# dmsuehir/unet_distributed

Measured on AMD Instinct MI355X. Metric: images/sec (whole node) 2D UNet BraTS 128×128×4 at 1/2/4/8 MI355X; Dice parity, higher is better.
Workload: dtype bf16; 1 GPU; model=unet2d-transposed (base 32, depth 4, 7760385 params), global_batch=1024, per_gpu_batch=1024, img_size=128, in_channels=4, parallelism=dp1, backend=native

## Files before the change

### unet_distributed_amd/csrc/kernels/conv_epilogue.h

```cpp
#pragma once
#include "common.h"
#include "conv_params.h"

namespace unet {

struct PixCoord {
  int n, d, h, w;
};

__device__ __forceinline__ PixCoord decompose(int q, int OD, int OH, int OW) {
  PixCoord c;
  c.w = q % OW;
  int t = q / OW;
  c.h = t % OH;
  t /= OH;
  c.d = t % OD;
  c.n = t / OD;
  return c;
}

enum { EPI_GENERIC = 0, EPI_FWD = 1, EPI_DGRAD = 2, EPI_STATS = 3, EPI_DGRAD_NORM = 4 };

template <int BM, int BN, int NTHR = 256>
constexpr int epi_lds_bytes() {
// ... 1 lines not shown
}

__device__ __forceinline__ size_t route_pix(const ConvFwdParams& p, int q, uint32_t& rk) {
  const int g = q / p.OW, w = q - g * p.OW;
  if (p.OD > 1) {
    const int s = g / p.OH, h = g - s * p.OH;
    rk = ((uint32_t)(s & 1) << 2) | ((uint32_t)(h & 1) << 1) | (uint32_t)(w & 1);
    return ((size_t)(s >> 1) * (p.OH >> 1) + (h >> 1)) * (p.OW >> 1) + (w >> 1);
  }
  rk = ((uint32_t)(g & 1) << 1) | (uint32_t)(w & 1);
  return (size_t)(g >> 1) * (p.OW >> 1) + (w >> 1);
}
__device__ __forceinline__ bool route_hit(uint32_t cw, int e, uint32_t rk, bool d3) {
  const uint32_t k = d3 ? (cw >> (3 * e)) & 7u : (cw >> (2 * e)) & 3u;
  return k == rk && ((cw >> (24 + e)) & 1u);
}

__host__ __device__ inline const char* conv_norm_epi_check(const ConvFwdParams& p) {
  if (!p.stats && !p.nz) return nullptr;
  if (!p.stats) return "conv_fwd: nz (dgrad-norm epilogue) needs a stats buffer";
  if (p.relu || p.shuffle || p.drop_rate > 0.f || p.out_scale != 1.f || p.D1 != p.Cout || p.mask1 || p.mask2 ||
      p.head_w || p.relu_bits || p.mask_bits || (p.route_gy && !p.nz))
    return "conv_fwd: statistics epilogue takes no ReLU / dropout / shuffle / scale / split / mask / head";
  if (p.nz && (p.bias || !p.na || !p.nc || p.npix <= 0 || p.mask_scale1 != 1.f || (p.ncs != 0 && p.ncs != p.Cout)))
    return "conv_fwd: dgrad-norm epilogue needs na / nc / npix, no bias";
  return nullptr;
}

__host__ __device__ inline int conv_epi_mode(const ConvFwdParams& p) {
  if (p.nz) return EPI_DGRAD_NORM;
  if (p.stats) return EPI_STATS;
  if (p.shuffle || p.drop_rate > 0.f || p.out_scale != 1.f) return EPI_GENERIC;
  if (p.relu && p.D1 == p.Cout && !p.mask1 && !p.mask2 && p.mask_scale1 == 1.f) return EPI_FWD;
  if (!p.relu && !p.bias) return EPI_DGRAD;
  return EPI_GENERIC;
}

template <int WM>
struct LinearTiles {
  __device__ static int base(int wm, int i) { return wm * WM + i * 16; }
};
template <int W, int RW, int TC, int NCS>
struct StripTiles {
  __device__ static int base(int wave, int i) {
    return ((wave / NCS) * RW + i / TC) * W + (wave % NCS) * 16 * TC + (i % TC) * 16;
  }
};

constexpr int kWaitVm0 = 0x0f70, kWaitLgkm0 = 0xc07f;
__device__ __forceinline__ void lds_barrier() {
  asm volatile("" ::: "memory");
  __builtin_amdgcn_s_waitcnt(kWaitLgkm0);
  __builtin_amdgcn_s_barrier();
  asm volatile("" ::: "memory");
}

template <int TN>
struct EpiConst {
  float bias[TN][4];
  float hw[8];
  float hb;
};

struct HeadWsum {
  float s[3][8];
  float u, v, w;
};
struct HeadT {
  float t[8];
  bool on;
};

template <int BM, int BN, int NTHR>
__device__ __forceinline__ void epi_mask_bits_load(const ConvFwdParams& p, const int m0, const int n0, const int tid,
                                                   uint32_t (&mb)[BM * (BN / 8) / NTHR]) {
  constexpr int CPR = BN / 8, NIT = BM * CPR / NTHR, RPI = NTHR / CPR;
  static_assert(BM * CPR % NTHR == 0 && NTHR % CPR == 0, "whole chunk passes");
  const int co = n0 + (tid % CPR) * 8, ml0 = tid / CPR;
#pragma unroll
  for (int it = 0; it < NIT; ++it)
    mb[it] = ((const uint8_t*)p.mask1)[((size_t)(m0 + ml0 + it * RPI) * p.D1 + co) >> 3];
}

template <int BM, int BN, int WM, int WN, int TM, int TN, int NTHR, int EPI = EPI_GENERIC,
          class MapM = LinearTiles<WM>, int SEGW = 0, int TROW = 0>
__device__ __forceinline__ HeadWsum conv_epilogue(const ConvFwdParams p, f32x4 (&acc)[TM][TN], char* smem,
                                                  const int m0, const int n0, const int M, const int wm,
                                                  const int wn, const int lane, const int tid,
                                                  const int pitch = 0, const int col0 = 0, const int stat_row = 0,
                                                  const EpiConst<TN>* ec = nullptr, const HeadT ht = HeadT{},
                                                  const uint32_t* pmb = nullptr) {
  HeadWsum hws;
#pragma unroll
  for (int k = 0; k < 3; ++k)
#pragma unroll
    for (int e = 0; e < 8; ++e) hws.s[k][e] = 0.f;
  hws.u = hws.v = hws.w = 0.f;
  auto qof = [&](int ml) -> int {
    if constexpr (SEGW > 0) return (m0 + ml / SEGW) * pitch + col0 + (ml % SEGW);
    else return m0 + ml;
  };
  constexpr bool ESWZ = BN == 32;
  constexpr int EPI_STRIDE = ESWZ ? 64 : (BN + 4) * 2;
  auto eoff = [](const int ml, const int chunk) -> int {
    return ESWZ ? ml * 64 + 16 * (chunk ^ ((ml >> 2) & 3)) : ml * EPI_STRIDE + 16 * chunk;
  };
  auto ehalf = [](const int ml, const int nl) -> int {
    return ESWZ ? ml * 64 + 16 * ((nl >> 3) ^ ((ml >> 2) & 3)) + ((2 * (nl & 7)) ^ (8 * ((ml >> 1) & 1)))
                : ml * EPI_STRIDE + 2 * nl;
  };
  auto eread = [&](const int ml, const int chunk) -> u32x4 {
    if constexpr (ESWZ) {
      const u32x4 v = *(const u32x4*)(smem + eoff(ml, chunk));
      return ((ml >> 1) & 1) ? (u32x4){v[2], v[3], v[0], v[1]} : v;
    } else {
      const u32x2 lo = *(const u32x2*)(smem + eoff(ml, chunk));
      const u32x2 hi = *(const u32x2*)(smem + eoff(ml, chunk) + 8);
      return (u32x4){lo[0], lo[1], hi[0], hi[1]};
    }
  };
  char* E = smem;
  float* SP = (float*)(smem + BM * EPI_STRIDE);
  constexpr bool G = EPI == EPI_GENERIC;
  constexpr bool kNormG = EPI == EPI_DGRAD_NORM;
  const bool kRelu = G ? (p.relu != 0) : (EPI == EPI_FWD);
  const bool kBias = EPI != EPI_DGRAD && !kNormG && p.bias;
  const bool kDrop = G && p.drop_rate > 0.f;
  constexpr bool kStats = EPI == EPI_STATS;
  const bool kShuffle = G && p.shuffle;
  constexpr bool kMaskScale = EPI == EPI_GENERIC || EPI == EPI_DGRAD;
  const float inv_keep = p.drop_rate > 0.f ? 1.f / (1.f - p.drop_rate) : 1.f;
  const uint32_t drop_thr = (uint32_t)(p.drop_rate * 4294967296.0);
  const uint32_t seed = (kDrop && p.seed_ptr) ? *p.seed_ptr : p.seed;
  const int Dtb = kShuffle ? (p.Cout >> p.shuffle) : p.Cout;
#pragma unroll
  for (int j = 0; j < TN; ++j) {
    const int nl = wn * WN + j * 16 + (lane >> 4) * 4;
    const int n = n0 + nl;
    float bsv[4], msc[4];
#pragma unroll
    for (int r = 0; r < 4; ++r) {
      bsv[r] = ec ? ec->bias[j][r] : (kBias ? p.bias[kShuffle ? (n + r) % Dtb : n + r] : 0.f);
      msc[r] = kMaskScale ? ((n + r < p.D1) ? p.mask_scale1 : p.mask_scale2) : 1.f;
    }
    if constexpr (EPI == EPI_FWD) {
      const f32x2 b01 = {bsv[0], bsv[1]}, b23 = {bsv[2], bsv[3]};
#pragma unroll
      for (int i = 0; i < TM; ++i) {
        const int ml = MapM::base(wm, i) + (lane & 15);
        f32x2 a01 = (f32x2){acc[i][j][0], acc[i][j][1]} + b01;
        f32x2 a23 = (f32x2){acc[i][j][2], acc[i][j][3]} + b23;
        u32x2 pk;
        pk[0] = relu2h(pack2h(a01[0], a01[1]));
        pk[1] = relu2h(pack2h(a23[0], a23[1]));
        *(u32x2*)(E + ehalf(ml, nl)) = pk;
      }
      continue;
    }
#pragma unroll
    for (int i = 0; i < TM; ++i) {
      const int ml = MapM::base(wm, i) + (lane & 15);
      const int q = qof(ml);
      float v[4];
#pragma unroll
      for (int r = 0; r < 4; ++r) {
        float x = G ? acc[i][j][r] * p.out_scale + bsv[r] : acc[i][j][r] + bsv[r];
        if (kRelu) x = fmaxf(x, 0.f);
        if (kDrop) {
          const uint32_t h = drop_hash((uint64_t)q * p.Cout + n + r + p.drop_idx0, seed, p.salt);
          x = (h >= drop_thr) ? x * inv_keep : 0.f;
        }
        if (kMaskScale) x *= msc[r];
        v[r] = x;
      }
      u32x2 pk;
      pk[0] = pack2h(v[0], v[1]);
      pk[1] = pack2h(v[2], v[3]);
      *(u32x2*)(E + ehalf(ml, nl)) = pk;
    }
  }
  if (pmb)
    lds_barrier();
  else
    __syncthreads();

  constexpr int CPR = BN / 8;
  constexpr int NCHUNK = BM * CPR;
  auto stats_out = [&](float (&s1)[8], float (&s2)[8], int cb) {
#pragma unroll
    for (int o = CPR; o < 64; o <<= 1)
#pragma unroll
      for (int e = 0; e < 8; ++e) {
        s1[e] += __shfl_xor(s1[e], o, 64);
        s2[e] += __shfl_xor(s2[e], o, 64);
      }
    const int wv = tid >> 6;
    if ((tid & 63) < CPR) {
#pragma unroll
      for (int e = 0; e < 8; ++e) {
        SP[(wv * 2 + 0) * BN + cb * 8 + e] = s1[e];
        SP[(wv * 2 + 1) * BN + cb * 8 + e] = s2[e];
      }
    }
    __syncthreads();
    for (int t = tid; t < 2 * BN; t += NTHR) {
      const int mom = t / BN, c = t - mom * BN;
      float a = 0.f;
#pragma unroll
      for (int w = 0; w < NTHR / 64; ++w) a += SP[(w * 2 + mom) * BN + c];
      p.stats[((size_t)stat_row * 2 + mom) * p.Cout + n0 + c] = a;
    }
  };
  if constexpr (kStats) {
    static_assert(NCHUNK % NTHR == 0 && NTHR % CPR == 0 && CPR <= 64, "statistics tiling");
    constexpr int NIT = NCHUNK / NTHR, RPI = NTHR / CPR;
    const int cb = tid % CPR, ml0 = tid / CPR;
    const int n = n0 + cb * 8;
    h16* dst = (h16*)p.dst1;
    float s1[8], s2[8];
#pragma unroll
    for (int e = 0; e < 8; ++e) s1[e] = s2[e] = 0.f;
#pragma unroll
    for (int it = 0; it < NIT; ++it) {
      const int ml = ml0 + it * RPI;
      const int q = qof(ml);
      if (q >= M) continue;
      const u32x4 v = eread(ml, cb);
      *(u32x4*)(dst + (size_t)q * p.Cout + n) = v;
      float f[8];
      unpack8(v, f);
#pragma unroll
      for (int e = 0; e < 8; ++e) {
        s1[e] += f[e];
        s2[e] = fmaf(f[e], f[e], s2[e]);
      }
    }
    stats_out(s1, s2, cb);
    return hws;
  }
  if constexpr (kNormG) {
    static_assert(NCHUNK % NTHR == 0 && NTHR % CPR == 0 && CPR <= 64, "dgrad-norm tiling");
    constexpr int NIT = NCHUNK / NTHR, RPI = NTHR / CPR;
    const int cb = tid % CPR, ml0 = tid / CPR;
    const int n = n0 + cb * 8;
    h16* dst = (h16*)p.dst1;
    const h16* zt = (const h16*)p.nz;
    const size_t crow = p.ncs ? (size_t)(qof(0) / p.npix) * p.ncs : 0;
    float ca[8], cc[8];
#pragma unroll
    for (int e = 0; e < 8; ++e) {
      ca[e] = p.na[crow + n + e];
      cc[e] = p.nc[crow + n + e];
    }
    u32x4 zv[NIT];
#pragma unroll
    for (int it = 0; it < NIT; ++it) {
      const int q = qof(ml0 + it * RPI);
      if (q < M) zv[it] = *(const u32x4*)(zt + (size_t)q * p.Cout + n);
    }
    const bool route = p.route_gy != nullptr, d3 = p.OD > 1;
    u32x4 rg[NIT];
    uint32_t rc[NIT], rk[NIT];
    if (route) {
      const int cpp = p.Cout >> 3;
#pragma unroll
      for (int it = 0; it < NIT; ++it) {
        const int q = qof(ml0 + it * RPI);
        if (q < M) {
          const size_t pq = route_pix(p, q, rk[it]);
          rc[it] = p.pool_code[pq * cpp + (n >> 3)];
          rg[it] = *(const u32x4*)((const h16*)p.route_gy + pq * p.Cout + n);
        }
      }
    }
    const bool drop = p.nd_rate > 0.f;
    const float dscale = drop ? 1.f / (1.f - p.nd_rate) : 1.f;
    const uint32_t dthr = (uint32_t)(p.nd_rate * 4294967296.0);
    const uint32_t dseed = p.seed_ptr ? *p.seed_ptr : p.seed;
    float s1[8], s2[8];
#pragma unroll
    for (int e = 0; e < 8; ++e) s1[e] = s2[e] = 0.f;
#pragma unroll
    for (int it = 0; it < NIT; ++it) {
      const int ml = ml0 + it * RPI;
      const int q = qof(ml);
      if (q >= M) continue;
      float g[8], z[8];
      unpack8(eread(ml, cb), g);
      unpack8(zv[it], z);
      if (route) {
        float gg[8];
        unpack8(rg[it], gg);
        const uint32_t cw = rc[it];
#pragma unroll
        for (int e = 0; e < 8; ++e)
          if (route_hit(cw, e, rk[it], d3)) g[e] += gg[e];
      }
#pragma unroll
      for (int e = 0; e < 8; ++e) {
        bool keep = fmaf(ca[e], z[e], cc[e]) > 0.f;
        if (drop) keep = keep && drop_hash((uint64_t)q * p.Cout + n + e, dseed, p.nd_salt) >= dthr;
        g[e] = keep ? g[e] * dscale : 0.f;
      }
      const u32x4 gv = pack8(g);
      *(u32x4*)(dst + (size_t)q * p.Cout + n) = gv;
      unpack8(gv, g);
#pragma unroll
      for (int e = 0; e < 8; ++e) {
        s1[e] += g[e];
        s2[e] = fmaf(g[e], z[e], s2[e]);
      }
    }
    stats_out(s1, s2, cb);
    return hws;
  }
  if constexpr (EPI == EPI_DGRAD && NCHUNK % NTHR == 0 && NTHR % CPR == 0) {
    constexpr int NIT = NCHUNK / NTHR, RPI = NTHR / CPR;
    const int cb = tid % CPR, ml0 = tid / CPR;
    const int n = n0 + cb * 8;
    const bool side1 = n < p.D1;
    const int rs = side1 ? p.D1 : p.Cout - p.D1;
    const int co = side1 ? n : n - p.D1;
    h16* dst = (h16*)(side1 ? p.dst1 : p.dst2);
    const h16* mk = (const h16*)(side1 ? p.mask1 : p.mask2);
    const bool mbit = (p.mask_bits >> (side1 ? 0 : 1)) & 1;
    u32x4 mv[NIT];
    uint32_t mb[NIT];
    if (mk && pmb) {
#pragma unroll
      for (int it = 0; it < NIT; ++it) mb[it] = pmb[it];
    } else if (mk) {
#pragma unroll
      for (int it = 0; it < NIT; ++it) {
        const int q = qof(ml0 + it * RPI);
        if (q < M) {
          if (mbit)
            mb[it] = ((const uint8_t*)mk)[((size_t)q * rs + co) >> 3];
          else
            mv[it] = *(const u32x4*)(mk + (size_t)q * rs + co);
        }
      }
    }
    const bool route = !pmb && p.route_gy != nullptr, d3 = p.OD > 1;
    u32x4 rg[NIT];
    uint32_t rc[NIT], rk[NIT];
    if (route) {
      const int cpp = p.Cout >> 3;
#pragma unroll
      for (int it = 0; it < NIT; ++it) {
        const int q = qof(ml0 + it * RPI);
        if (q < M) {
          const size_t pq = route_pix(p, q, rk[it]);
          rc[it] = p.pool_code[pq * cpp + (n >> 3)];
          rg[it] = *(const u32x4*)((const h16*)p.route_gy + pq * p.Cout + n);
        }
      }
    }
#pragma unroll
    for (int it = 0; it < NIT; ++it) {
      const int ml = ml0 + it * RPI;
      const int q = qof(ml);
      if (q >= M) continue;
      u32x4 v = eread(ml, cb);
      if (mk) v = (mbit || pmb) ? keep_bits(v, mb[it]) : keep_pos(v, mv[it]);
      if (route) {
        float o[8], gg[8];
        unpack8(v, o);
        unpack8(rg[it], gg);
        const uint32_t cw = rc[it];
#pragma unroll
        for (int e = 0; e < 8; ++e)
          if (route_hit(cw, e, rk[it], d3)) o[e] += gg[e];
        v = pack8(o);
      }
      *(u32x4*)(dst + (size_t)q * rs + co) = v;
    }
    return hws;
  }
  const int Dt = kShuffle ? (p.Cout >> p.shuffle) : 0;
  constexpr bool kHeadable = EPI == EPI_FWD && BN == 32 && NTHR % CPR == 0;
  const bool kHead = kHeadable && p.head_w != nullptr;
  float hw[8], hb = 0.f;
  constexpr int HIT = kHeadable ? NCHUNK / NTHR : 1;
  static_assert(!kHeadable || (NCHUNK % NTHR == 0 && HIT % CPR == 0 && HIT <= 8), "fused head tiling");
  float hz[HIT];
  int hq[HIT];
#pragma unroll
  for (int k = 0; k < HIT; ++k) {
    hz[k] = 0.f;
    hq[k] = M;
  }
  if (kHeadable && kHead) {
#pragma unroll
    for (int e = 0; e < 8; ++e) hw[e] = ec ? ec->hw[e] : p.head_w[(tid % CPR) * 8 + e];
    hb = ec ? ec->hb : p.head_b[0];
  }
  constexpr int NITER = (NCHUNK + NTHR - 1) / NTHR;
  constexpr int UNR = kHeadable ? NITER : 2;
#pragma unroll UNR
  for (int it = 0; it < NITER; ++it) {
    const int c = tid + it * NTHR;
    if (NCHUNK % NTHR && c >= NCHUNK) break;
    const int ml = c / CPR, cb = c % CPR;
    const int q = qof(ml);
    if (q >= M) continue;
    const int n = n0 + cb * 8;
    u32x4 v = eread(ml, cb);
    size_t off;
    h16* dst;
    const void* mk;
    bool mbit = false;
    if (EPI == EPI_FWD || EPI == EPI_STATS) {
      off = (size_t)q * p.Cout + n;
      dst = (h16*)p.dst1;
      mk = nullptr;
    } else if (kShuffle) {
      const int tap = n / Dt, co = n - tap * Dt;
      const PixCoord pc = decompose(q, p.OD, p.OH, p.OW);
      int td = 0, th, tw;
      if (p.shuffle == 3) {
        td = tap >> 2;
        th = (tap >> 1) & 1;
        tw = tap & 1;
      } else {
        th = tap >> 1;
        tw = tap & 1;
      }
      const int dd = p.shuffle == 3 ? 2 : 1;
      const size_t pix = (((size_t)pc.n * (p.OD * dd) + pc.d * dd + td) * (2 * p.OH) + 2 * pc.h + th) *
                             (2 * p.OW) + 2 * pc.w + tw;
      off = pix * Dt + co;
      dst = (h16*)p.dst1;
      mk = p.mask1;
      mbit = p.mask_bits & 1;
    } else if (n < p.D1) {
      off = (size_t)q * p.D1 + n;
      dst = (h16*)p.dst1;
      mk = p.mask1;
      mbit = p.mask_bits & 1;
    } else {
      off = (size_t)q * (p.Cout - p.D1) + (n - p.D1);
      dst = (h16*)p.dst2;
      mk = p.mask2;
      mbit = (p.mask_bits >> 1) & 1;
    }
    if (EPI != EPI_FWD && EPI != EPI_STATS && mk) {
      v = mbit ? keep_bits(v, ((const uint8_t*)mk)[off >> 3]) : keep_pos(v, *(const u32x4*)((const h16*)mk + off));
// ... 95 lines not shown
```

### unet_distributed_amd/csrc/kernels/conv_win.h

```cpp
#pragma once
#include "common.h"
#include "conv_params.h"
#include "conv_epilogue.h"
#include "head_grad.h"
#include <type_traits>

namespace unet {

enum { GEO_2D = 0, GEO_SEG = 1, GEO_3D = 2 };

inline int win_bn(const ConvFwdParams& p) {
  if (p.tile == 12) return 64;
  if (p.tile == 6) return 32;
  const int W = p.OW > 128 ? 128 : p.OW;
  return (p.Cout % 64 == 0 && W <= 64 && !p.head_w) ? 64 : 32;
}
inline int win_bm(const ConvFwdParams& p) {
  const int W = p.OW > 128 ? 128 : p.OW;
  return (W == 16 || win_bn(p) == 64) ? 256 : 512;
}
inline int win_rows(const ConvFwdParams& p) {
  const int W = p.OW > 128 ? 128 : p.OW;
  return win_bm(p) / W;
}
// ... 455 lines not shown
        float xa[8], xb[8];
#pragma unroll
        for (int e = 0; e < 8; ++e) {
          const size_t ci = xsample + cb + xlc * 8 + e;
          xa[e] = p.xa[ci];
          xb[e] = p.xb[ci];
        }
        const bool xdrop = p.xd_rate > 0.f;
        const uint32_t xseed = xdrop ? (p.seed_ptr ? *p.seed_ptr : p.seed) : 0u;
        const float xinv = xdrop ? 1.f / (1.f - p.xd_rate) : 1.f;
        const uint32_t xthr = (uint32_t)(p.xd_rate * 4294967296.0);
#pragma unroll
        for (int j = 0; j < XNJ; ++j) {
          int hr, hc, gr;
          bool ok;
          const int sl = xslot(j, hr, hc, gr, ok);
          if (!ok) continue;
          char* a = Xs + sl * 64 + 16 * (xlc ^ ((hc >> 1) & 3));
          float v[8];
          unpack8(*(const u32x4*)a, v);
#pragma unroll
          for (int e = 0; e < 8; ++e) v[e] = fmaxf(fmaf(xa[e], v[e], xb[e]), 0.f);
          if (xdrop) {
            const unsigned long long e0 = p.xd_idx0 + (unsigned long long)(gr * W + hc - 1) * C + cb + xlc * 8;
#pragma unroll
            for (int e = 0; e < 8; ++e) v[e] = drop_hash(e0 + e, xseed, p.xd_salt) >= xthr ? v[e] * xinv : 0.f;
          }
          const u32x4 o = pack8(v);
          *(u32x4*)a = o;
          if (p.xout && tn == 0 && hr >= 1 && hr <= R)
            *(u32x4*)((h16*)p.xout + (size_t)(gr * W + hc - 1) * C + cb + xlc * 8) = o;
        }
        __syncthreads();
      }
      chunk_mfmas(XF == 4 ? s2d_taps : 0x1ffu);
    }
  }
  __syncthreads();
  if constexpr (GEO == GEO_SEG)
    conv_epilogue<BM, BN, WMP, BN, TM, TN, NTHR, EPI, Map, W, W>(p, acc, smem, g0, n0, M, wave, 0, lane, tid, Wf,
                                                                 col0, tm);
  else if constexpr (GEO == GEO_2D)
    conv_epilogue<BM, BN, WMP, BN, TM, TN, NTHR, EPI, Map, 0, W>(p, acc, smem, g0 * W, n0, M, wave, 0, lane, tid, 0, 0,
                                                                  tm);
  else
    conv_epilogue<BM, BN, WMP, BN, TM, TN, NTHR, EPI, Map>(p, acc, smem, g0 * W, n0, M, wave, 0, lane, tid, 0, 0, tm);
}

constexpr int PF_HWP = 144;
constexpr int PF_ROWB = PF_HWP * 64;
constexpr int PF_CPT = 6 * 128 * 4 / NTHR;
constexpr int PF_XB = 6 * PF_ROWB, PF_WB = 9 * 32 * 64;
static_assert(512 * 36 * 2 <= PF_XB, "epilogue staging aliases the halo image");

__device__ __forceinline__ void head_ws_store(HeadWsum& hws, char* smem, const int wave, const int lane,
                                              const int tid, float* row) {
#pragma unroll
  for (int k = 0; k < 3; ++k)
#pragma unroll
    for (int e = 0; e < 8; ++e)
#pragma unroll
      for (int o = 4; o < 64; o <<= 1) hws.s[k][e] += __shfl_xor(hws.s[k][e], o, 64);
  hws.u = wave_sum(hws.u);
  hws.v = wave_sum(hws.v);
  hws.w = wave_sum(hws.w);
  float* red = (float*)smem;
  __syncthreads();
  if (lane < 4) {
#pragma unroll
    for (int k = 0; k < 3; ++k)
#pragma unroll
      for (int e = 0; e < 8; ++e) red[wave * 100 + k * 32 + lane * 8 + e] = hws.s[k][e];
  }
  if (lane == 0) {
    red[wave * 100 + 96] = hws.u;
    red[wave * 100 + 97] = hws.v;
    red[wave * 100 + 98] = hws.w;
    red[wave * 100 + 99] = 0.f;
  }
  __syncthreads();
  if (tid < 100) row[tid] = (red[tid] + red[100 + tid]) + (red[200 + tid] + red[300 + tid]);
}

template <int EPI, int XF, int GEO = GEO_2D>
__global__ void __launch_bounds__(NTHR, 2) conv_win_pf_kernel(const ConvFwdParams p) {
  static_assert(XF == 0 || (XF == 3 && EPI == EPI_DGRAD && GEO == GEO_2D) || (XF == 1 && GEO == GEO_2D),
                "plain source, head-on-load data gradient or normalise on load");
  static_assert(GEO == GEO_2D || GEO == GEO_SEG, "2D rows");
  constexpr bool SEG = GEO == GEO_SEG;
  constexpr int W = 128, R = 4, BM = 512, BN = 32, ROWB = PF_ROWB;
  constexpr int TC = 2, NCS = 4, RW = 4, TM = RW * TC, TN = 2, WMP = BM / 4;
  using Map = StripTiles<W, RW, TC, NCS>;
  __shared__ __attribute__((aligned(1024))) char smem[PF_XB + PF_WB];
  char* Xs = smem;
  char* Ws = smem + PF_XB;
  const int tid = threadIdx.x, lane = tid & 63, wave = __builtin_amdgcn_readfirstlane(tid >> 6);
  const int H = p.OH;
  const int Wf = SEG ? p.OW : W;
  const int nseg = SEG ? p.OW / W : 1;
  const int rows_total = p.N * H;
  const int M = rows_total * Wf;
  const int nwin = rows_total / R * nseg;
  const int w_lo = (int)blockIdx.x * p.win_pf;
  const int w_hi = w_lo + p.win_pf < nwin ? w_lo + p.win_pf : nwin;
  if (w_lo >= w_hi) return;
  constexpr int OOB = 0x7fffffff;
  const char* src = (const char*)p.src1;

  u32x4 hv[PF_CPT], ev = {0u, 0u, 0u, 0u};
  const int gl_t = tid * 16;
  const int lds_t = (1 + (tid >> 2)) * 64 + 16 * ((tid & 3) ^ (((1 + (tid >> 2)) >> 1) & 3));
  constexpr int NSL = 6 * PF_HWP, HJ = (NSL + NTHR - 1) / NTHR;
  float hpr[HJ], htv[HJ];
  uint32_t hbits[HJ];
  HeadGradCtx hctx{};
  if constexpr (XF == 3) hctx = head_grad_ctx(p.hg);
  float xan[8], xbn[8];
  int pf_g0 = 0;
  bool pf_top = false, pf_bot = false;
  constexpr bool HWS = EPI == EPI_FWD && !SEG;
  float tnext[HWS ? 8 : 1];
  auto load_halo = [&](const int w) {
    const int tmw = p.rev ? nwin - 1 - w : w;
    const int g0 = (tmw / nseg) * R, col0 = (tmw % nseg) * W;
    if constexpr (HWS) {
      if (p.head_ws) {
#pragma unroll
        for (int it = 0; it < 8; ++it) tnext[it] = bits2f(((const uint16_t*)p.head_t)[g0 * W + (tid >> 2) + 64 * it]);
      }
    }
    if constexpr (XF == 3) {
      const bool top_in = (g0 % H) != 0, bot_in = ((g0 + R) % H) != 0;
#pragma unroll
      for (int j = 0; j < HJ; ++j) {
        const int sl = tid + NTHR * j;
        const int hr = sl / PF_HWP, hc = sl - hr * PF_HWP;
        const int gr = g0 - 1 + hr, col = hc - 1;
        const bool ok = sl < NSL && (hr > 0 || top_in) && (hr < R + 1 || bot_in) &&
                        (unsigned)gr < (unsigned)rows_total && (unsigned)col < (unsigned)W;
        const int pix = ok ? gr * W + col : 0;
        hpr[j] = p.hg.prob[pix];
        htv[j] = bits2f(((const uint16_t*)p.hg.t)[pix]);
        hbits[j] = ok ? ((const uint32_t*)p.hg.bits)[pix] : 0u;
      }
      return;
    }
    const int grow0 = (g0 / H) * H;
    const bool top_in = (g0 % H) != 0, bot_in = ((g0 + R) % H) != 0;
    if constexpr (XF == 1) {
      const size_t cs = (size_t)(g0 / H) * p.xcs + (tid & 3) * 8;
#pragma unroll
      for (int e = 0; e < 8; ++e) {
        xan[e] = p.xa[cs + e];
        xbn[e] = p.xb[cs + e];
      }
      pf_g0 = g0;
      pf_top = top_in;
      pf_bot = bot_in;
    }
    const __amdgpu_buffer_rsrc_t rs =
        __builtin_amdgcn_make_buffer_rsrc((void*)(src + (size_t)grow0 * Wf * 64), (short)0, OOB, 0x00020000);
    const int rowoff = ((g0 - 1 - grow0) * Wf + col0) * 64;
#pragma unroll
    for (int c = 0; c < PF_CPT; ++c) {
      const int hr = c >> 1;
      const bool ok = (hr > 0 || top_in) && (hr < R + 1 || bot_in) && (unsigned)(g0 - 1 + hr) < (unsigned)rows_total;
      hv[c] = __builtin_amdgcn_raw_buffer_load_b128(rs, ok ? rowoff + hr * Wf * 64 + (c & 1) * 4096 + gl_t : OOB, 0, 0);
    }
    if constexpr (SEG) {
      const int hr = tid >> 3, col = ((tid >> 2) & 1) ? col0 + W : col0 - 1;
      const bool ok = tid < 48 && (hr > 0 || top_in) && (hr < R + 1 || bot_in) &&
                      (unsigned)(g0 - 1 + hr) < (unsigned)rows_total && (unsigned)col < (unsigned)Wf;
      ev = __builtin_amdgcn_raw_buffer_load_b128(
          rs, ok ? ((g0 - 1 + hr - grow0) * Wf + col) * 64 + (tid & 3) * 16 : OOB, 0, 0);
    }
  };
  auto store_halo = [&]() {
    if constexpr (XF == 3) {
#pragma unroll
      for (int j = 0; j < HJ; ++j) {
        const int sl = tid + NTHR * j;
        if (sl >= NSL) continue;
        const int hc = sl % PF_HWP;
        const float dz = head_dlogit(hpr[j], htv[j], hctx.a, hctx.bb, hctx.inv_total, hctx.bce_w, hctx.gscale);
        const int sw = (hc >> 1) & 3;
#pragma unroll
        for (int k = 0; k < 4; ++k) {
          float o[8];
#pragma unroll
          for (int e = 0; e < 8; ++e) {
            const float v = dz * hctx.w[8 * k + e];
            o[e] = ((hbits[j] >> (8 * k + e)) & 1u) ? v : 0.f;
          }
          *(u32x4*)(Xs + sl * 64 + 16 * (k ^ sw)) = pack8(o);
        }
      }
      return;
    }
    if constexpr (XF == 1) {
#pragma unroll
      for (int c = 0; c < PF_CPT; ++c) {
        const int hr = c >> 1;
        const int gr = pf_g0 - 1 + hr;
        u32x4 v = hv[c];
        if ((hr > 0 || pf_top) && (hr < R + 1 || pf_bot) && (unsigned)gr < (unsigned)rows_total) {
          float f[8];
          unpack8(v, f);
#pragma unroll
          for (int e = 0; e < 8; ++e) f[e] = fmaxf(fmaf(xan[e], f[e], xbn[e]), 0.f);
          v = pack8(f);
          if (p.xout && hr >= 1 && hr <= R)
            *(u32x4*)((h16*)p.xout + ((size_t)gr * W + (tid >> 2) + 64 * (c & 1)) * 32 + (tid & 3) * 8) = v;
        }
        *(u32x4*)(Xs + lds_t + hr * ROWB + (c & 1) * 4096) = v;
      }
    } else {
#pragma unroll
      for (int c = 0; c < PF_CPT; ++c) *(u32x4*)(Xs + lds_t + (c >> 1) * ROWB + (c & 1) * 4096) = hv[c];
    }
    if (tid < 48) *(u32x4*)(Xs + (tid >> 3) * ROWB + ((tid >> 2) & 1) * 129 * 64 + 16 * (tid & 3)) = ev;
  };
  load_halo(w_lo);
  {
    const __amdgpu_buffer_rsrc_t rsw = __builtin_amdgcn_make_buffer_rsrc((void*)p.wgt, (short)0, OOB, 0x00020000);
    const int lslot = lane >> 2;
    const int lchunk = (lane & 3) ^ ((lslot >> 1) & 3);
    const int wl = (lslot * p.Kpad + lchunk * 8) * 2;
    constexpr int WI = 9 * BN / 16;
#pragma unroll
    for (int q = 0; q < (WI + 3) / 4; ++q) {
      const int k = wave + 4 * q;
      if (k < WI) {
        const int tap = k / (BN / 16), nb = (k % (BN / 16)) * 16;
        __builtin_amdgcn_raw_ptr_buffer_load_lds(rsw, (__attribute__((address_space(3))) void*)(Ws + k * 1024), 16,
                                                 (nb * p.Kpad + tap * 32) * 2 + wl, 0, 0, 0);
      }
    }
  }
  const int fsub = lane >> 4, fr = lane & 15;
  EpiConst<TN> ec;
#pragma unroll
  for (int j = 0; j < TN; ++j)
#pragma unroll
    for (int r = 0; r < 4; ++r)
      ec.bias[j][r] = (EPI != EPI_DGRAD && EPI != EPI_DGRAD_NORM && p.bias) ? p.bias[16 * j + 4 * fsub + r] : 0.f;
#pragma unroll
  for (int e = 0; e < 8; ++e) ec.hw[e] = (EPI == EPI_FWD && p.head_w) ? p.head_w[(tid % 4) * 8 + e] : 0.f;
  ec.hb = (EPI == EPI_FWD && p.head_w) ? p.head_b[0] : 0.f;
  HeadWsum hws;
#pragma unroll
  for (int k = 0; k < 3; ++k)
#pragma unroll
    for (int e = 0; e < 8; ++e) hws.s[k][e] = 0.f;
  hws.u = hws.v = hws.w = 0.f;
  HeadT ht;
  ht.on = HWS && p.head_ws;
#pragma unroll
  for (int it = 0; it < 8; ++it) ht.t[it] = HWS ? tnext[it] : 0.f;
  store_halo();
  __syncthreads();

  const int r0 = (wave / NCS) * RW, c0 = (wave % NCS) * 16 * TC;
  int xbase[3];
#pragma unroll
  for (int dw = 0; dw < 3; ++dw) {
    const int hc = fr + dw;
    xbase[dw] = r0 * ROWB + c0 * 64 + hc * 64 + 16 * (fsub ^ ((hc >> 1) & 3));
  }
  const int wbase = fr * 64 + 16 * (fsub ^ ((fr >> 1) & 3));
  for (int w = w_lo; w < w_hi; ++w) {
    const int tm = p.rev ? nwin - 1 - w : w;
    const int g0 = (tm / nseg) * R, col0 = (tm % nseg) * W;
    if (w + 1 < w_hi) load_halo(w + 1);
    f32x4 acc[TM][TN];
#pragma unroll
    for (int i = 0; i < TM; ++i)
#pragma unroll
      for (int j = 0; j < TN; ++j) acc[i][j] = (f32x4){0.f, 0.f, 0.f, 0.f};
#pragma unroll
    for (int dw = 0; dw < 3; ++dw) {
      h16x8 wf[3][TN];
#pragma unroll
      for (int dh = 0; dh < 3; ++dh)
#pragma unroll
        for (int j = 0; j < TN; ++j) wf[dh][j] = *(const h16x8*)(Ws + ((3 * dh + dw) * BN + 16 * j) * 64 + wbase);
#pragma unroll
      for (int hr = 0; hr < RW + 2; ++hr) {
#pragma unroll
        for (int ci = 0; ci < TC; ++ci) {
          const h16x8 xf = *(const h16x8*)(Xs + xbase[dw] + hr * ROWB + ci * 16 * 64);
#pragma unroll
          for (int dh = 0; dh < 3; ++dh) {
            const int ri = hr - dh;
            if (ri < 0 || ri >= RW) continue;
#pragma unroll
            for (int j = 0; j < TN; ++j) acc[ri * TC + ci][j] = mfma16(wf[dh][j], xf, acc[ri * TC + ci][j]);
          }
        }
      }
    }
    __syncthreads();
    if constexpr (SEG)
      conv_epilogue<BM, BN, WMP, BN, TM, TN, NTHR, EPI, Map, W, W>(p, acc, smem, g0, 0, M, wave, 0, lane, tid, Wf,
                                                                    col0, tm, &ec);
    else {
      const HeadWsum r = conv_epilogue<BM, BN, WMP, BN, TM, TN, NTHR, EPI, Map, 0, W>(
          p, acc, smem, g0 * W, 0, M, wave, 0, lane, tid, 0, 0, tm, &ec, ht);
      if constexpr (HWS) {
#pragma unroll
        for (int k = 0; k < 3; ++k)
#pragma unroll
          for (int e = 0; e < 8; ++e) hws.s[k][e] += r.s[k][e];
        hws.u += r.u;
        hws.v += r.v;
        hws.w += r.w;
      }
    }
    if (w + 1 < w_hi) {
      __syncthreads();
      store_halo();
      if constexpr (HWS) {
#pragma unroll
        for (int it = 0; it < 8; ++it) ht.t[it] = tnext[it];
      }
      __syncthreads();
    }
  }
  if constexpr (EPI == EPI_FWD && !SEG) {
    if (p.head_ws) head_ws_store(hws, smem, wave, lane, tid, p.head_ws + (size_t)blockIdx.x * 100);
  }
}

template <int W, bool CONCAT, int EPI, bool DZ = false>
__global__ void __launch_bounds__(NTHR, 2) conv_win_cp_kernel(const ConvFwdParams p) {
  constexpr int BN = 64, BM = 256, R = BM / W, HR = R + 2;
  constexpr int HWP = W + 4, ROWB = HWP * 64;
  constexpr int NSLOT = HR * HWP;
  constexpr int XB = (NSLOT + 15) / 16 * 1024, WB = 9 * BN * 64;
  constexpr int XG = (NSLOT * 4 + NTHR - 1) / NTHR;
  constexpr int WG = 9 * BN * 4 / NTHR;
  constexpr int EPIB = (EPI == EPI_STATS || EPI == EPI_DGRAD_NORM) ? epi_lds_bytes<BM, BN>() : BM * (BN + 4) * 2;
  constexpr int KB = DZ ? 3 * CP_DZ_MAXC * 4 : 0;
  constexpr int LDS_BYTES = (XB + WB + KB > EPIB) ? XB + WB + KB : EPIB;
  constexpr int WMP = BM / 4, TM = WMP / 16, TN = BN / 16;
  constexpr int TC = 1, NCS = W / 16, RW = R / (4 / NCS);
  static_assert(W >= 16 && W <= 64 && RW * TC == TM && 9 * BN * 4 % NTHR == 0, "chunk-pipelined window shape");
  using Map = StripTiles<W, RW, TC, NCS>;
  __shared__ __attribute__((aligned(1024))) char smem[LDS_BYTES];
  char* Xs = smem;
  char* Ws = smem + XB;
  const int tid = threadIdx.x, lane = tid & 63, wave = __builtin_amdgcn_readfirstlane(tid >> 6);
  const int H = p.OH;
  const int rows_total = p.N * H;
  const int M = rows_total * W;
  const int tiles_n = p.Cout / BN;
  const int bid = xcd_remap(blockIdx.x, gridDim.x);
  const int tm0 = bid / tiles_n, tn = bid % tiles_n;
  const int tm = p.rev ? (int)(gridDim.x / tiles_n) - 1 - tm0 : tm0;
  const int g0 = tm * R, n0 = tn * BN;
  const int Cin = p.C1 + p.C2;
  const int nchunks = Cin >> 5;
  constexpr int OOB = 0x7fffffff;
  const int grow0 = (g0 / H) * H;
  const size_t img_px = (size_t)grow0 * W;
  const char* s1b = (const char*)p.src1 + img_px * p.C1 * 2;
  const char* s2b = p.src2 ? (const char*)p.src2 + img_px * p.C2 * 2 : s1b;
  const __amdgpu_buffer_rsrc_t rs1 = __builtin_amdgcn_make_buffer_rsrc((void*)s1b, (short)0, OOB, 0x00020000);
  const __amdgpu_buffer_rsrc_t rs2 = __builtin_amdgcn_make_buffer_rsrc((void*)s2b, (short)0, OOB, 0x00020000);
  const __amdgpu_buffer_rsrc_t rsw = __builtin_amdgcn_make_buffer_rsrc((void*)p.wgt, (short)0, OOB, 0x00020000);
  const bool top_in = (g0 % H) != 0, bot_in = ((g0 + R) % H) != 0;
  float* Ks = (float*)(smem + XB + WB);
  const __amdgpu_buffer_rsrc_t rsz = __builtin_amdgcn_make_buffer_rsrc(
      (void*)(DZ ? (const char*)p.xz + img_px * p.C1 * 2 : s1b), (short)0, OOB, 0x00020000);
  if constexpr (DZ) {
    const size_t xs = (size_t)(g0 / H) * p.xcs;
    for (int i = tid; i < 3 * Cin; i += NTHR) {
      const int m = i / Cin, c = i - m * Cin;
      Ks[i] = (m == 0 ? p.xa : m == 1 ? p.xb : p.xc)[xs + c];
    }
  }

  u32x4 xv[XG], wv[WG];
  u32x4 zq[DZ ? XG : 1];
  uint32_t okm = 0;
  auto load_chunk = [&](const int kc) {
    const bool from1 = !CONCAT || (kc << 5) < p.C1;
    const int C = from1 ? p.C1 : p.C2;
    const int cb = from1 ? (kc << 5) : (kc << 5) - p.C1;
    const __amdgpu_buffer_rsrc_t rs = from1 ? rs1 : rs2;
#pragma unroll
    for (int c = 0; c < XG; ++c) {
      const int u = tid + NTHR * c;
      const int sl = u >> 2, hr = sl / HWP, hc = sl - hr * HWP;
      const int gr = g0 - 1 + hr, col = hc - 1;
      const bool ok = sl < NSLOT && (hr > 0 || top_in) && (hr < R + 1 || bot_in) &&
                      (unsigned)gr < (unsigned)rows_total && (unsigned)col < (unsigned)W;
      xv[c] = __builtin_amdgcn_raw_buffer_load_b128(
          rs, ok ? (((gr - grow0) * W + col) * C + cb + (u & 3) * 8) * 2 : OOB, 0, 0);
      if constexpr (DZ) {
        zq[c] = __builtin_amdgcn_raw_buffer_load_b128(
            rsz, ok ? (((gr - grow0) * W + col) * C + cb + (u & 3) * 8) * 2 : OOB, 0, 0);
        okm = c ? (okm | ((ok ? 1u : 0u) << c)) : (ok ? 1u : 0u);
      }
    }
#pragma unroll
    for (int c = 0; c < WG; ++c)
      wv[c] = __builtin_amdgcn_raw_buffer_load_b128(
// ... 467 lines not shown
#pragma unroll
      for (int hr = 0; hr < RW + 2; ++hr) {
#pragma unroll
        for (int ci = 0; ci < TC; ++ci) {
          const h16x8 xf = *(const h16x8*)(Xs + xbase[dw] + hr * ROWB + ci * 16 * 64);
#pragma unroll
          for (int dh = 0; dh < 3; ++dh) {
            const int ri = hr - dh;
            if (ri < 0 || ri >= RW) continue;
#pragma unroll
            for (int j = 0; j < TN; ++j) acc[ri * TC + ci][j] = mfma16(wf[dh][j], xf, acc[ri * TC + ci][j]);
          }
        }
      }
    }
  };
  load_coarse(w_lo);
  load_skip(w_lo);
  for (int w = w_lo; w < w_hi; ++w) {
    const int tm = p.rev ? nwin - 1 - w : w;
    const int g0 = tm * R;
#pragma unroll
    for (int i = 0; i < TM; ++i)
#pragma unroll
      for (int j = 0; j < TN; ++j) acc[i][j] = (f32x4){0.f, 0.f, 0.f, 0.f};
    form_u();
    if (w + 1 < w_hi) load_coarse(w + 1);
    __syncthreads();
    chunk_mfmas(Wu);
    __syncthreads();
    store_skip();
    if (w + 1 < w_hi) load_skip(w + 1);
    __syncthreads();
    chunk_mfmas(Wk);
    __syncthreads();
    conv_epilogue<BM, BN, WMP, BN, TM, TN, NTHR, EPI, Map, 0, W>(p, acc, smem, g0 * W, 0, M, wave, 0, lane, tid, 0, 0,
                                                                  tm, &ec);
    __syncthreads();
  }
}

hipError_t launch_win_pfu(const ConvFwdParams& p, hipStream_t s) {
  const int grid = win_grid(p);
  const bool st = conv_epi_mode(p) == EPI_STATS;
  if (p.ut.C == 64 && st)
    UNET_LAUNCH((conv_win_pfu_kernel<2, EPI_STATS>), dim3(grid), dim3(NTHR), 0, s, p);
  else if (p.ut.C == 64)
    UNET_LAUNCH((conv_win_pfu_kernel<2, EPI_FWD>), dim3(grid), dim3(NTHR), 0, s, p);
  else if (st)
    UNET_LAUNCH((conv_win_pfu_kernel<1, EPI_STATS>), dim3(grid), dim3(NTHR), 0, s, p);
  else
    UNET_LAUNCH((conv_win_pfu_kernel<1, EPI_FWD>), dim3(grid), dim3(NTHR), 0, s, p);
  return launch_status();
}

hipError_t launch_win_pf(const ConvFwdParams& p, hipStream_t s) {
  const int grid = win_grid(p);
  if (p.OW > 128) {
    switch (conv_epi_mode(p)) {
      case EPI_FWD: UNET_LAUNCH((conv_win_pf_kernel<EPI_FWD, 0, GEO_SEG>), dim3(grid), dim3(NTHR), 0, s, p); break;
      case EPI_DGRAD: UNET_LAUNCH((conv_win_pf_kernel<EPI_DGRAD, 0, GEO_SEG>), dim3(grid), dim3(NTHR), 0, s, p); break;
      case EPI_STATS: UNET_LAUNCH((conv_win_pf_kernel<EPI_STATS, 0, GEO_SEG>), dim3(grid), dim3(NTHR), 0, s, p); break;
      case EPI_DGRAD_NORM:
        UNET_LAUNCH((conv_win_pf_kernel<EPI_DGRAD_NORM, 0, GEO_SEG>), dim3(grid), dim3(NTHR), 0, s, p);
        break;
      default: UNET_LAUNCH((conv_win_pf_kernel<EPI_GENERIC, 0, GEO_SEG>), dim3(grid), dim3(NTHR), 0, s, p); break;
    }
    return launch_status();
  }
  if (p.xform) {
    if (conv_epi_mode(p) == EPI_STATS)
      UNET_LAUNCH((conv_win_pf_kernel<EPI_STATS, 1>), dim3(grid), dim3(NTHR), 0, s, p);
    else if (conv_epi_mode(p) == EPI_GENERIC)
      UNET_LAUNCH((conv_win_pf_kernel<EPI_GENERIC, 1>), dim3(grid), dim3(NTHR), 0, s, p);
    else
      return hipErrorInvalidValue;
    return launch_status();
  }
  switch (conv_epi_mode(p)) {
    case EPI_FWD: UNET_LAUNCH((conv_win_pf_kernel<EPI_FWD, 0>), dim3(grid), dim3(NTHR), 0, s, p); break;
    case EPI_DGRAD:
      if (p.hg.prob)
        UNET_LAUNCH((conv_win_pf_kernel<EPI_DGRAD, 3>), dim3(grid), dim3(NTHR), 0, s, p);
      else
        UNET_LAUNCH((conv_win_pf_kernel<EPI_DGRAD, 0>), dim3(grid), dim3(NTHR), 0, s, p);
      break;
    case EPI_STATS: UNET_LAUNCH((conv_win_pf_kernel<EPI_STATS, 0>), dim3(grid), dim3(NTHR), 0, s, p); break;
    case EPI_DGRAD_NORM: UNET_LAUNCH((conv_win_pf_kernel<EPI_DGRAD_NORM, 0>), dim3(grid), dim3(NTHR), 0, s, p); break;
    default: UNET_LAUNCH((conv_win_pf_kernel<EPI_GENERIC, 0>), dim3(grid), dim3(NTHR), 0, s, p); break;
  }
  return launch_status();
}

}

template <int BN, int BM>
hipError_t launch_win(const ConvFwdParams& p, hipStream_t s) {
  if constexpr (BN == 32 && BM == 512) {
    if (win_pf_eligible(p)) return launch_win_pf(p, s);
    if (win_pfu_eligible(p)) return launch_win_pfu(p, s);
    if (win_cp128_eligible(p)) return launch_win_cp128(p, s);
  }
  if constexpr (BN == 64 && BM == 256) {
    if (win_cp_eligible(p)) return launch_win_cp(p, s);
  }
  const int W = p.OW > 128 ? 128 : p.OW;
  const int grid = win_grid(p);
  const bool cc = p.C2 > 0;
  const int epi = conv_epi_mode(p);
  const int geo = p.KD == 3 ? GEO_3D : (p.OW > W ? GEO_SEG : GEO_2D);
#define WIN_EPI(WW, CC, GG)                                                                               \
  if (epi == EPI_FWD)                                                                                     \
    UNET_LAUNCH((conv_win_kernel<WW, BN, BM, CC, EPI_FWD, GG>), dim3(grid), dim3(NTHR), 0, s, p);     \
  else if (epi == EPI_DGRAD)                                                                              \
    UNET_LAUNCH((conv_win_kernel<WW, BN, BM, CC, EPI_DGRAD, GG>), dim3(grid), dim3(NTHR), 0, s, p);   \
  else if (epi == EPI_STATS)                                                                              \
    UNET_LAUNCH((conv_win_kernel<WW, BN, BM, CC, EPI_STATS, GG>), dim3(grid), dim3(NTHR), 0, s, p);   \
  else if (epi == EPI_DGRAD_NORM && !CC)                                                                  \
    UNET_LAUNCH((conv_win_kernel<WW, BN, BM, false, EPI_DGRAD_NORM, GG>), dim3(grid), dim3(NTHR), 0, s, p); \
  else if (epi == EPI_DGRAD_NORM)                                                                         \
    return hipErrorInvalidValue;                                                                          \
  else                                                                                                    \
    UNET_LAUNCH((conv_win_kernel<WW, BN, BM, CC, EPI_GENERIC, GG>), dim3(grid), dim3(NTHR), 0, s, p);
#define WIN_GEO(WW, CC)                                                                                   \
  if (geo == GEO_3D) {                                                                                    \
    WIN_EPI(WW, CC, GEO_3D)                                                                               \
  } else {                                                                                                \
    WIN_EPI(WW, CC, GEO_2D)                                                                               \
  }
#define WIN_CASE(WW)                                                                                      \
  case WW:                                                                                                \
    if constexpr (win_tile_built<BN, BM>(WW)) {                                                           \
      if (cc) {                                                                                           \
        WIN_GEO(WW, true)                                                                                 \
      } else {                                                                                            \
        WIN_GEO(WW, false)                                                                                \
      }                                                                                                   \
    } else {                                                                                              \
      return hipErrorInvalidValue;                                                                        \
    }                                                                                                     \
    break;
#define XF_CASE(WW)                                                                                           \
  case WW:                                                                                                    \
    if constexpr (win_tile_built<BN, BM>(WW)) {                                                               \
      if (p.xform == 2) {                                                                                     \
        if constexpr ((BN == 64 && BM == 256 && WW <= 64) || (BN == 32 && BM == 512 && WW == 64)) {           \
          if (epi == EPI_DGRAD_NORM)                                                                          \
            UNET_LAUNCH((conv_win_kernel<WW, BN, BM, false, EPI_DGRAD_NORM, GEO_2D, 2>), dim3(grid), dim3(NTHR), 0, s, \
                        p);                                                                                   \
          else if (epi == EPI_DGRAD)                                                                          \
            UNET_LAUNCH((conv_win_kernel<WW, BN, BM, false, EPI_DGRAD, GEO_2D, 2>), dim3(grid), dim3(NTHR), 0, s, p); \
          else                                                                                                \
            return hipErrorInvalidValue;                                                                      \
        } else {                                                                                              \
          return hipErrorInvalidValue;                                                                        \
        }                                                                                                     \
      } else if (epi == EPI_STATS)                                                                            \
        UNET_LAUNCH((conv_win_kernel<WW, BN, BM, false, EPI_STATS, GEO_2D, 1>), dim3(grid), dim3(NTHR), 0, s, p); \
      else if (epi == EPI_GENERIC)                                                                            \
        UNET_LAUNCH((conv_win_kernel<WW, BN, BM, false, EPI_GENERIC, GEO_2D, 1>), dim3(grid), dim3(NTHR), 0, s, p); \
      else                                                                                                    \
        return hipErrorInvalidValue;                                                                          \
    } else {                                                                                                  \
      return hipErrorInvalidValue;                                                                            \
    }                                                                                                         \
    break;
// ... 114 lines not shown
```

Before: 49140 images/sec.

## Preload dgrad epilogue mask bits and pool-route operands before the window MMA loop

```diff
diff --git a/unet_distributed_amd/csrc/kernels/conv_epilogue.h b/unet_distributed_amd/csrc/kernels/conv_epilogue.h
--- a/unet_distributed_amd/csrc/kernels/conv_epilogue.h
+++ b/unet_distributed_amd/csrc/kernels/conv_epilogue.h
@@ -107,6 +107,32 @@
     mb[it] = ((const uint8_t*)p.mask1)[((size_t)(m0 + ml0 + it * RPI) * p.D1 + co) >> 3];
 }
 
+template <int NIT>
+struct EpiPre {
+  uint32_t mb[NIT > 0 ? NIT : 1];
+  uint32_t rc[NIT > 1 ? NIT / 2 : 1];
+  u32x4 rg[NIT > 1 ? NIT / 2 : 1];
+  bool on;
+  bool route;
+};
+template <int BM, int BN, int NTHR, int TROW>
+__device__ __forceinline__ void epi_pre_load(const ConvFwdParams& p, const int m0, const int n0, const int tid,
+                                             EpiPre<BM * (BN / 8) / NTHR>& pre) {
+  constexpr int CPR = BN / 8, NIT = BM * CPR / NTHR, RPI = NTHR / CPR;
+  static_assert(TROW == 2 * RPI && NIT % 4 == 0 && (BM / TROW) % 2 == 0, "two chunk passes per row, whole row pairs");
+  epi_mask_bits_load<BM, BN, NTHR>(p, m0, n0, tid, pre.mb);
+  if (pre.route) {
+    const int n = n0 + (tid % CPR) * 8, ml0 = tid / CPR;
+    const int prow = (m0 / TROW) >> 1;
+#pragma unroll
+    for (int r = 0; r < NIT / 2; ++r) {
+      const size_t pq = (size_t)(prow + (r >> 1)) * (TROW / 2) + ((ml0 + (r & 1) * RPI) >> 1);
+      pre.rc[r] = p.pool_code[pq * (p.Cout >> 3) + (n >> 3)];
+      pre.rg[r] = *(const u32x4*)((const h16*)p.route_gy + pq * p.Cout + n);
+    }
+  }
+}
+
 template <int BM, int BN, int WM, int WN, int TM, int TN, int NTHR, int EPI = EPI_GENERIC,
           class MapM = LinearTiles<WM>, int SEGW = 0, int TROW = 0>
 __device__ __forceinline__ HeadWsum conv_epilogue(const ConvFwdParams p, f32x4 (&acc)[TM][TN], char* smem,
@@ -114,7 +140,8 @@
                                                   const int wn, const int lane, const int tid,
                                                   const int pitch = 0, const int col0 = 0, const int stat_row = 0,
                                                   const EpiConst<TN>* ec = nullptr, const HeadT ht = HeadT{},
-                                                  const uint32_t* pmb = nullptr) {
+                                                  const uint32_t* pmb = nullptr,
+                                                  const EpiPre<BM * (BN / 8) / NTHR>* pre = nullptr) {
   HeadWsum hws;
 #pragma unroll
   for (int k = 0; k < 3; ++k)
@@ -204,7 +231,8 @@
       *(u32x2*)(E + ehalf(ml, nl)) = pk;
     }
   }
-  if (pmb)
+  const bool pre_on = pre != nullptr && pre->on;
+  if (pmb || pre_on)
     lds_barrier();
   else
     __syncthreads();
@@ -354,6 +382,9 @@
     if (mk && pmb) {
 #pragma unroll
       for (int it = 0; it < NIT; ++it) mb[it] = pmb[it];
+    } else if (mk && pre_on) {
+#pragma unroll
+      for (int it = 0; it < NIT; ++it) mb[it] = pre->mb[it];
     } else if (mk) {
 #pragma unroll
       for (int it = 0; it < NIT; ++it) {
@@ -366,10 +397,20 @@
         }
       }
     }
-    const bool route = !pmb && p.route_gy != nullptr, d3 = p.OD > 1;
+    const bool route = pre_on ? pre->route : (!pmb && p.route_gy != nullptr), d3 = p.OD > 1;
     u32x4 rg[NIT];
     uint32_t rc[NIT], rk[NIT];
-    if (route) {
+    if (route && pre_on) {
+      if constexpr (TROW > 0 && SEGW == 0 && NIT % 4 == 0) {
+#pragma unroll
+        for (int it = 0; it < NIT; ++it) {
+          const int q = qof(ml0 + it * RPI);
+          rk[it] = ((uint32_t)((q / TROW) & 1) << 1) | (uint32_t)(q & 1);
+          rc[it] = pre->rc[2 * (it >> 2) + (it & 1)];
+          rg[it] = pre->rg[2 * (it >> 2) + (it & 1)];
+        }
+      }
+    } else if (route) {
       const int cpp = p.Cout >> 3;
 #pragma unroll
       for (int it = 0; it < NIT; ++it) {
@@ -387,7 +428,7 @@
       const int q = qof(ml);
       if (q >= M) continue;
       u32x4 v = eread(ml, cb);
-      if (mk) v = (mbit || pmb) ? keep_bits(v, mb[it]) : keep_pos(v, mv[it]);
+      if (mk) v = (mbit || pmb || pre_on) ? keep_bits(v, mb[it]) : keep_pos(v, mv[it]);
       if (route) {
         float o[8], gg[8];
         unpack8(v, o);
diff --git a/unet_distributed_amd/csrc/kernels/conv_win.h b/unet_distributed_amd/csrc/kernels/conv_win.h
--- a/unet_distributed_amd/csrc/kernels/conv_win.h
+++ b/unet_distributed_amd/csrc/kernels/conv_win.h
@@ -561,10 +561,11 @@
   if (tid < 100) row[tid] = (red[tid] + red[100 + tid]) + (red[200 + tid] + red[300 + tid]);
 }
 
-template <int EPI, int XF, int GEO = GEO_2D>
+template <int EPI, int XF, int GEO = GEO_2D, int PRE = 0>
 __global__ void __launch_bounds__(NTHR, 2) conv_win_pf_kernel(const ConvFwdParams p) {
   static_assert(XF == 0 || (XF == 3 && EPI == EPI_DGRAD && GEO == GEO_2D) || (XF == 1 && GEO == GEO_2D),
                 "plain source, head-on-load data gradient or normalise on load");
+  static_assert(PRE == 0 || (EPI == EPI_DGRAD && XF == 0 && GEO == GEO_2D), "preloaded epilogue operands");
   static_assert(GEO == GEO_2D || GEO == GEO_SEG, "2D rows");
   constexpr bool SEG = GEO == GEO_SEG;
   constexpr int W = 128, R = 4, BM = 512, BN = 32, ROWB = PF_ROWB;
@@ -598,16 +599,22 @@
   int pf_g0 = 0;
   bool pf_top = false, pf_bot = false;
   constexpr bool HWS = EPI == EPI_FWD && !SEG;
-  float tnext[HWS ? 8 : 1];
-  auto load_halo = [&](const int w) {
+  uint32_t tnext[2] = {0u, 0u};
+  auto take_targets = [&](HeadT& ht) {
+#pragma unroll
+    for (int it = 0; it < 8; ++it) {
+      const int src = (it & 1) ? (int)tnext[1] : (int)tnext[0];
+      const int k = it >> 1;
+      const int b = k == 0   ? __builtin_amdgcn_mov_dpp(src, 0x00, 0xf, 0xf, true)
+                    : k == 1 ? __builtin_amdgcn_mov_dpp(src, 0x55, 0xf, 0xf, true)
+                    : k == 2 ? __builtin_amdgcn_mov_dpp(src, 0xaa, 0xf, 0xf, true)
+                             : __builtin_amdgcn_mov_dpp(src, 0xff, 0xf, 0xf, true);
+      ht.t[it] = bits2f((uint16_t)b);
+    }
+  };
+  auto load_halo = [&](const int w, const bool valid = true) {
     const int tmw = p.rev ? nwin - 1 - w : w;
     const int g0 = (tmw / nseg) * R, col0 = (tmw % nseg) * W;
-    if constexpr (HWS) {
-      if (p.head_ws) {
-#pragma unroll
-        for (int it = 0; it < 8; ++it) tnext[it] = bits2f(((const uint16_t*)p.head_t)[g0 * W + (tid >> 2) + 64 * it]);
-      }
-    }
     if constexpr (XF == 3) {
       const bool top_in = (g0 % H) != 0, bot_in = ((g0 + R) % H) != 0;
 #pragma unroll
@@ -637,8 +644,8 @@
       pf_top = top_in;
       pf_bot = bot_in;
     }
-    const __amdgpu_buffer_rsrc_t rs =
-        __builtin_amdgcn_make_buffer_rsrc((void*)(src + (size_t)grow0 * Wf * 64), (short)0, OOB, 0x00020000);
+    const __amdgpu_buffer_rsrc_t rs = __builtin_amdgcn_make_buffer_rsrc((void*)(src + (size_t)grow0 * Wf * 64), (short)0,
+                                                                        valid ? OOB : 0, 0x00020000);
     const int rowoff = ((g0 - 1 - grow0) * Wf + col0) * 64;
 #pragma unroll
     for (int c = 0; c < PF_CPT; ++c) {
@@ -652,6 +659,13 @@
                       (unsigned)(g0 - 1 + hr) < (unsigned)rows_total && (unsigned)col < (unsigned)Wf;
       ev = __builtin_amdgcn_raw_buffer_load_b128(
           rs, ok ? ((g0 - 1 + hr - grow0) * Wf + col) * 64 + (tid & 3) * 16 : OOB, 0, 0);
+    }
+    if constexpr (HWS) {
+      if (p.head_ws) {
+        const uint16_t* tp = (const uint16_t*)p.head_t + g0 * W + (tid >> 2) + 128 * (tid & 3);
+        tnext[0] = tp[0];
+        tnext[1] = tp[64];
+      }
     }
   };
   auto store_halo = [&]() {
@@ -735,7 +749,8 @@
   HeadT ht;
   ht.on = HWS && p.head_ws;
 #pragma unroll
-  for (int it = 0; it < 8; ++it) ht.t[it] = HWS ? tnext[it] : 0.f;
+  for (int it = 0; it < 8; ++it) ht.t[it] = 0.f;
+  if constexpr (HWS) take_targets(ht);
   store_halo();
   __syncthreads();
 
@@ -747,10 +762,18 @@
     xbase[dw] = r0 * ROWB + c0 * 64 + hc * 64 + 16 * (fsub ^ ((hc >> 1) & 3));
   }
   const int wbase = fr * 64 + 16 * (fsub ^ ((fr >> 1) & 3));
+  EpiPre<BM * (BN / 8) / NTHR> pre;
+  pre.on = PRE > 0;
+  pre.route = PRE > 1;
   for (int w = w_lo; w < w_hi; ++w) {
     const int tm = p.rev ? nwin - 1 - w : w;
     const int g0 = (tm / nseg) * R, col0 = (tm % nseg) * W;
-    if (w + 1 < w_hi) load_halo(w + 1);
+    if constexpr (PRE > 0) {
+      epi_pre_load<BM, BN, NTHR, W>(p, g0 * W, 0, tid, pre);
+      load_halo(w + 1, w + 1 < w_hi);
+    } else {
+      if (w + 1 < w_hi) load_halo(w + 1);
+    }
     f32x4 acc[TM][TN];
 #pragma unroll
     for (int i = 0; i < TM; ++i)
@@ -784,7 +807,7 @@
                                                                     col0, tm, &ec);
     else {
       const HeadWsum r = conv_epilogue<BM, BN, WMP, BN, TM, TN, NTHR, EPI, Map, 0, W>(
-          p, acc, smem, g0 * W, 0, M, wave, 0, lane, tid, 0, 0, tm, &ec, ht);
+          p, acc, smem, g0 * W, 0, M, wave, 0, lane, tid, 0, 0, tm, &ec, ht, nullptr, &pre);
       if constexpr (HWS) {
 #pragma unroll
         for (int k = 0; k < 3; ++k)
@@ -795,13 +818,10 @@
         hws.w += r.w;
       }
     }
-    if (w + 1 < w_hi) {
+    if (PRE > 0 || w + 1 < w_hi) {
       __syncthreads();
       store_halo();
-      if constexpr (HWS) {
-#pragma unroll
-        for (int it = 0; it < 8; ++it) ht.t[it] = tnext[it];
-      }
+      if constexpr (HWS) take_targets(ht);
       __syncthreads();
     }
   }
@@ -1435,6 +1455,10 @@
     case EPI_DGRAD:
       if (p.hg.prob)
         UNET_LAUNCH((conv_win_pf_kernel<EPI_DGRAD, 3>), dim3(grid), dim3(NTHR), 0, s, p);
+      else if (p.mask1 && (p.mask_bits & 1) && p.D1 == p.Cout && p.route_gy)
+        UNET_LAUNCH((conv_win_pf_kernel<EPI_DGRAD, 0, GEO_2D, 2>), dim3(grid), dim3(NTHR), 0, s, p);
+      else if (p.mask1 && (p.mask_bits & 1) && p.D1 == p.Cout)
+        UNET_LAUNCH((conv_win_pf_kernel<EPI_DGRAD, 0, GEO_2D, 1>), dim3(grid), dim3(NTHR), 0, s, p);
       else
         UNET_LAUNCH((conv_win_pf_kernel<EPI_DGRAD, 0>), dim3(grid), dim3(NTHR), 0, s, p);
       break;
```

After: 49560 images/sec, median of 6. Within noise of the previous version (+0.9%).
